# beehive-lab/GPULlama3.java

Measured on AMD Instinct MI355X. Metric: tg128 tok/s (llama-bench), Llama-3-8B Q8_0, higher is better.
Workload: dtype i8; 1 GPU; Llama-3-8B-random Q8_0 random-weight GGUF-layout model, tg128 at depth 0 (one step = 128 decode tokens, logits D2H inside the timed region); parallelism=single GPU, ranks=1, ctx=648

## Files before the change

### gpullama3.java_amd/csrc/gl3_api.hip

```cpp
#include <chrono>
#include <cstdio>
#include <cstdlib>
#include <cstring>
#include <vector>

#include "gl3_ctx.h"
#include "gl3_batch_plan.h"
#include "gl3_decode_kernels.h"
#include "gl3_rowlane_kernels.h"
#include "gl3_veclane_kernels.h"
#include "gl3_moe_kernels.h"
#include "gl3_kv_copy.h"

using namespace gl3;

static std::string g_create_err;

static double now_ms() {
    return std::chrono::duration<double, std::milli>(std::chrono::steady_clock::now().time_since_epoch()).count();
}


static size_t matvec_smem(int pro, int epi, const Q8Mat& w) {
    const int nm = epi == EPI_SWIGLU ? 2 : 1;
    return (size_t)w.ng * 4 * 32 + (size_t)w.ng * 4 * 4 + (pro == PRO_RMS ? (size_t)(w.k + 32) * 4 : 0) + (size_t)2 * nm * w.ng * 64 * 4 + 128;
}

#include <hip/hip_ext.h>
template <typename K>
static void launch_mv(gl3_ctx* ctx, K kernel, int wgs, int threads, size_t smem, const MatvecArgs& a) {
    if (ctx->prof_ev0) hipExtLaunchKernelGGL(kernel, dim3(wgs), dim3(threads), (uint32_t)smem, ctx->stream, ctx->prof_ev0, ctx->prof_ev1, 0, a);
    else hipLaunchKernelGGL(kernel, dim3(wgs), dim3(threads), smem, ctx->stream, a);
}

template <int PRO, int EPI>
static void launch_matvec_t(gl3_ctx* ctx, const MatvecArgs& a, int wgs, size_t smem, bool nt) {
    if (a.tp) { launch_mv(ctx, matvec_q8t_kernel<PRO, EPI, true, 4, false, true>, wgs, mv_threads(4), smem, a); return; }
    if (nt) launch_mv(ctx, matvec_q8t_kernel<PRO, EPI, true>, wgs, mv_threads(4), smem, a);
    else launch_mv(ctx, matvec_q8t_kernel<PRO, EPI, false>, wgs, mv_threads(4), smem, a);
}

template <int PRO, int EPI>
static hipError_t allow_big_lds() {
    hipError_t e = hipFuncSetAttribute((const void*)matvec_q8t_kernel<PRO, EPI, true>, hipFuncAttributeMaxDynamicSharedMemorySize, 160 * 1024 - 256);
    if (e != hipSuccess) return e;
    e = hipFuncSetAttribute((const void*)matvec_q8t_kernel<PRO, EPI, true, 4, false, true>, hipFuncAttributeMaxDynamicSharedMemorySize, 160 * 1024 - 256);
    if (e != hipSuccess) return e;
    return hipFuncSetAttribute((const void*)matvec_q8t_kernel<PRO, EPI, false>, hipFuncAttributeMaxDynamicSharedMemorySize, 160 * 1024 - 256);
}

static void launch_matvec(gl3_ctx* ctx, int pro, int epi, const Q8Mat& w, const Q8Mat* w2, const float* x,
                          const float* norm_w, float* out, const float* resid_in, float out_scale = 1.0f, const TpRec* tp = nullptr) {
    if (w.fmt != GL3_TYPE_Q8_0) {
        hipStream_t s = ctx->stream;
        static const bool vl_rms = env_flag("GL3_VL_RMS", true);
        static const bool ksplit_on = env_flag("GL3_VLQ", true);
        const bool ksplit_type = ksplit_on && w.vl && (w.fmt == GL3_FMT_Q8V || w.fmt == GL3_TYPE_Q4_0);
        const long vl_waves = (long)((w.rows + 7) / 8) * (epi == EPI_SWIGLU ? 2 : 1);
        const bool fuse_rms = pro == PRO_RMS && w.vl && vl_rms && vl_rms_fusable(w.k) && epi != EPI_RESID && !(ksplit_type && vl_waves <= 512);
        if (pro == PRO_RMS && !fuse_rms) {
            const size_t sm = (size_t)(w.k + 32) * 4 + ss_scratch_bytes(w.k) + 64;
            hipLaunchKernelGGL(rmsnorm_f32_kernel, dim3(1), dim3(256), sm, s, x, w.k, norm_w, ctx->d.rms_eps, ctx->xn);
            x = ctx->xn;
        }
        if (w.vl) {
            VlArgs v{};
            v.w = w.w; v.w2 = w2 ? w2->w : nullptr; v.rows = w.rows; v.k = w.k; v.x = x; v.out = out; v.resid_in = resid_in; v.out_scale = out_scale;
            v.tp = tp;
            const dim3 vg(((w.rows + 7) / 8 + VL_WAVES - 1) / VL_WAVES), vb(64 * VL_WAVES);
            const size_t vs = vl_smem_bytes(w.k);
            if (fuse_rms) {
                v.norm_w = norm_w; v.eps = ctx->d.rms_eps;
                const dim3 rg(((w.rows + 7) / 8 + VL_RMS_WAVES - 1) / VL_RMS_WAVES), rb(64 * VL_RMS_WAVES);
                const size_t rs = vl_rms_smem_bytes(w.k);
#define GL3_VLR(WT_) \
                do { \
                    if (epi == EPI_STORE) hipLaunchKernelGGL((matvec_vl_kernel<WT_, EPI_STORE, true, VL_RMS_WAVES>), rg, rb, rs, s, v); \
                    else hipLaunchKernelGGL((matvec_vl_kernel<WT_, EPI_SWIGLU, true, VL_RMS_WAVES>), rg, rb, rs, s, v); \
                } while (0)
                if (w.fmt == GL3_TYPE_F16 && (ctx->d.flags & GL3_FLAG_VECTOR_512)) {
                    if (epi == EPI_STORE) hipLaunchKernelGGL((matvec_vl_kernel<WT_F16, EPI_STORE, true, VL_RMS_WAVES, 512>), rg, rb, rs, s, v);
                    else hipLaunchKernelGGL((matvec_vl_kernel<WT_F16, EPI_SWIGLU, true, VL_RMS_WAVES, 512>), rg, rb, rs, s, v);
                }
                else if (w.fmt == GL3_TYPE_F16) GL3_VLR(WT_F16); else if (w.fmt == GL3_FMT_Q8V) GL3_VLR(WT_Q8_0); else GL3_VLR(WT_Q4_0);
#undef GL3_VLR
                return;
            }
#define GL3_VL(WT_) \
            do { \
                if (epi == EPI_STORE) hipLaunchKernelGGL((matvec_vl_kernel<WT_, EPI_STORE>), vg, vb, vs, s, v); \
                else if (epi == EPI_RESID) hipLaunchKernelGGL((matvec_vl_kernel<WT_, EPI_RESID>), vg, vb, vs, s, v); \
                else hipLaunchKernelGGL((matvec_vl_kernel<WT_, EPI_SWIGLU>), vg, vb, vs, s, v); \
            } while (0)
            static const bool ksplit = env_flag("GL3_VLQ", true);
#define GL3_VLQ_E(WT_, MAXW_) \
            do { \
                const size_t qs = vq_smem_bytes<WT_, MAXW_>(w.k, epi == EPI_SWIGLU ? 2 : 1, nw); \
                if (epi == EPI_STORE) hipLaunchKernelGGL((matvec_vlq_kernel<WT_, EPI_STORE, MAXW_>), qg, qb, qs, s, v); \
                else if (epi == EPI_RESID) hipLaunchKernelGGL((matvec_vlq_kernel<WT_, EPI_RESID, MAXW_>), qg, qb, qs, s, v); \
                else hipLaunchKernelGGL((matvec_vlq_kernel<WT_, EPI_SWIGLU, MAXW_>), qg, qb, qs, s, v); \
            } while (0)
#define GL3_VLQ(WT_) \
            do { \
                const int ngroups = (w.rows + 7) / 8, nw = vq_waves<WT_>(w.k, epi == EPI_SWIGLU ? 2 : 1, ngroups); \
                const dim3 qg(ngroups), qb(64 * nw); \
                if (nw == 16) GL3_VLQ_E(WT_, 16); else GL3_VLQ_E(WT_, 8); \
            } while (0)
            if (w.fmt == GL3_TYPE_F16 && (ctx->d.flags & GL3_FLAG_VECTOR_512)) {
                if (epi == EPI_STORE) hipLaunchKernelGGL((matvec_vl_kernel<WT_F16, EPI_STORE, false, VL_WAVES, 512>), vg, vb, vs, s, v);
                else if (epi == EPI_RESID) hipLaunchKernelGGL((matvec_vl_kernel<WT_F16, EPI_RESID, false, VL_WAVES, 512>), vg, vb, vs, s, v);
                else hipLaunchKernelGGL((matvec_vl_kernel<WT_F16, EPI_SWIGLU, false, VL_WAVES, 512>), vg, vb, vs, s, v);
            }
            else if (w.fmt == GL3_TYPE_F16) GL3_VL(WT_F16);
            else if (w.fmt == GL3_FMT_Q8V) { if (ksplit) GL3_VLQ(WT_Q8_0); else GL3_VL(WT_Q8_0); }
            else { if (ksplit) GL3_VLQ(WT_Q4_0); else GL3_VL(WT_Q4_0); }
#undef GL3_VLQ
#undef GL3_VLQ_E
#undef GL3_VL
            return;
        }
        RlArgs a{};
        a.w = w.w; a.w2 = w2 ? w2->w : nullptr; a.rows = w.rows; a.k = w.k; a.x = x; a.out = out; a.resid_in = resid_in; a.out_scale = out_scale;
        const dim3 grid((w.rows + 63) / 64);
        const size_t sm = rl_smem_bytes(w.k, epi);
#define GL3_RL(WT_) \
        do { \
            if (epi == EPI_STORE) hipLaunchKernelGGL((matvec_rl_kernel<WT_, EPI_STORE>), grid, dim3(RL_THREADS), sm, s, a); \
            else if (epi == EPI_RESID) hipLaunchKernelGGL((matvec_rl_kernel<WT_, EPI_RESID>), grid, dim3(RL_THREADS), sm, s, a); \
            else hipLaunchKernelGGL((matvec_rl_kernel<WT_, EPI_SWIGLU>), grid, dim3(RL_THREADS), sm, s, a); \
        } while (0)
        if (w.fmt == GL3_TYPE_F16) GL3_RL(WT_F16); else GL3_RL(WT_Q4_0);
#undef GL3_RL
        return;
    }
    static const bool nt = env_flag("GL3_NT", true);
    static const int max_wgs = getenv("GL3_WGS") ? atoi(getenv("GL3_WGS")) : 512;
    MatvecArgs a{};
    a.w = w.w; a.w2 = w2 ? w2->w : nullptr; a.rows = w.rows; a.k = w.k; a.ng = w.ng; a.nstrips = w.nstrips;
    a.x = x; a.norm_w = norm_w; a.eps = ctx->d.rms_eps; a.out = out; a.resid_in = resid_in; a.out_scale = out_scale;
    a.tp = tp;
    const int wgs = w.nstrips < max_wgs ? w.nstrips : max_wgs;
    const size_t smem = matvec_smem(pro, epi, w);
    if (pro == PRO_RMS && epi == EPI_STORE) launch_matvec_t<PRO_RMS, EPI_STORE>(ctx, a, wgs, smem, nt);
    else if (pro == PRO_QUANT && epi == EPI_RESID) {
        static const int wide_max = getenv("GL3_WIDE_STRIPS") ? atoi(getenv("GL3_WIDE_STRIPS")) : 256;
        if (w.nstrips <= wide_max && nt && tp)
            launch_mv(ctx, matvec_q8t_kernel<PRO_QUANT, EPI_RESID, true, 8, false, true>, wgs, mv_threads(8), smem, a);
        else if (w.nstrips <= wide_max && nt)
            launch_mv(ctx, matvec_q8t_kernel<PRO_QUANT, EPI_RESID, true, 8>, wgs, mv_threads(8), smem, a);
        else launch_matvec_t<PRO_QUANT, EPI_RESID>(ctx, a, wgs, smem, nt);
    }
    else launch_matvec_t<PRO_RMS, EPI_SWIGLU>(ctx, a, wgs, smem, nt);
}

static void launch_matvec_sel(gl3_ctx* ctx, int layer, int which, const Q8Mat& stack, const Q8Mat* stack2, int rows, const float* x,
                              const float* norm_w, float* out, int shared_rows) {
    const gl3_model_desc& d = ctx->d;
    static const int max_wgs = getenv("GL3_WGS") ? atoi(getenv("GL3_WGS")) : 512;
    Q8Mat sub = stack;
    sub.rows = rows; sub.nstrips = rows / 16;
    MatvecArgs a{};
    a.w = stack.w; a.w2 = stack2 ? stack2->w : nullptr; a.rows = rows; a.k = stack.k; a.ng = stack.ng; a.nstrips = sub.nstrips;
    a.x = x; a.norm_w = norm_w; a.eps = d.rms_eps; a.out = out; a.resid_in = nullptr; a.out_scale = 1.0f;
    a.moe = reinterpret_cast<const MoeSlots*>(ctx->moe_slots) + (size_t)layer * 3 + which;
    const int slots = d.n_experts_used + (which == 0 ? (shared_rows + rows - 1) / rows : 0);
    const int wgs = sub.nstrips < max_wgs ? sub.nstrips : max_wgs;
    const dim3 grid(wgs, slots);
    if (which != 2) hipLaunchKernelGGL((matvec_q8t_kernel<PRO_RMS, EPI_SWIGLU, true, 4, true>), grid, dim3(mv_threads(4)), matvec_smem(PRO_RMS, EPI_SWIGLU, sub), ctx->stream, a);
    else hipLaunchKernelGGL((matvec_q8t_kernel<PRO_QUANT, EPI_RESID, true, 4, true>), grid, dim3(mv_threads(4)), matvec_smem(PRO_QUANT, EPI_RESID, sub), ctx->stream, a);
}

static int32_t moe_build_slots(gl3_ctx* ctx) {
    const gl3_model_desc& d = ctx->d;
    std::vector<MoeSlots> h((size_t)d.n_layers * 3);
    for (int l = 0; l < d.n_layers; ++l) {
        const gl3_layer& L = ctx->layers[l];
        MoeSlots gu{};
        gu.sel = ctx->moe_sel; gu.sel_stride = (size_t)(d.moe_hidden / 16) * L.gate_exps.ng * TILE_BYTES;
        gu.x_slot_stride = 0; gu.out_slot_stride = d.moe_hidden; gu.n_sel = d.n_experts_used;
        gu.sh_rows = L.w1.rows; gu.sh_w = L.w1.w; gu.sh_w2 = L.w3.w; gu.sh_out = ctx->hb;
        h[(size_t)l * 3 + 0] = gu;
        gu.sh_rows = 0; gu.sh_w = gu.sh_w2 = nullptr; gu.sh_out = nullptr;
        h[(size_t)l * 3 + 1] = gu;
        MoeSlots dn{};
        dn.sel = ctx->moe_sel; dn.sel_stride = (size_t)(d.dim / 16) * L.down_exps.ng * TILE_BYTES;
        dn.x_slot_stride = d.moe_hidden; dn.out_slot_stride = d.dim; dn.n_sel = d.n_experts_used;
        h[(size_t)l * 3 + 2] = dn;
    }
    GL3_HIP(hipMalloc(&ctx->moe_slots, h.size() * sizeof(MoeSlots)));
    GL3_HIP(hipMemcpy(ctx->moe_slots, h.data(), h.size() * sizeof(MoeSlots), hipMemcpyHostToDevice));
    return GL3_OK;
}

struct Prof {
    gl3_ctx* ctx; gl3_kernel_times* kt; size_t n = 0; std::vector<int> klass;
    bool ext = false;
    void begin(int k, uint64_t bytes, bool single_kernel = false) {
        if (!kt) return;
        if (ctx->ev.size() < 2 * (n + 1)) {
            ctx->ev.resize(2 * (n + 1));
            hipEventCreate(&ctx->ev[2 * n]); hipEventCreate(&ctx->ev[2 * n + 1]);
        }
        ext = single_kernel;
        if (ext) { ctx->prof_ev0 = ctx->ev[2 * n]; ctx->prof_ev1 = ctx->ev[2 * n + 1]; }
        else hipEventRecord(ctx->ev[2 * n], ctx->stream);
        klass.push_back(k); kt->launches[k]++; kt->bytes[k] += bytes;
    }
    void end() {
        if (!kt) return;
        if (ext) ctx->prof_ev0 = ctx->prof_ev1 = nullptr;
        else hipEventRecord(ctx->ev[2 * n + 1], ctx->stream);
        ++n;
    }
    void collect() {
        if (!kt) return;
        hipStreamSynchronize(ctx->stream);
        for (size_t i = 0; i < n; ++i) {
            float ms = 0; hipEventElapsedTime(&ms, ctx->ev[2 * i], ctx->ev[2 * i + 1]);
            kt->ms[klass[i]] += ms;
        }
    }
};

static uint64_t mv_bytes(const Q8Mat& w) { return w.algo_bytes() + (uint64_t)w.k * 4 + (uint64_t)w.rows * 4; }

static void enqueue_moe_ffn(gl3_ctx* ctx, int l, Prof& pr) {
    gl3_layer& L = ctx->layers[l];
    const gl3_model_desc& d = ctx->d;
    hipStream_t s = ctx->stream;
    const int E = d.n_experts, topk = d.n_experts_used, mh = d.moe_hidden;
// ... 354 lines not shown
    ctx->q_dim = d.n_heads * d.head_size; ctx->kv_dim = d.n_kv_heads * d.head_size;
    ctx->heads_l = d.n_heads / tp; ctx->kv_heads_l = d.n_kv_heads / tp;
    ctx->q_dim_l = ctx->heads_l * d.head_size; ctx->kv_dim_l = ctx->kv_heads_l * d.head_size;
    ctx->hidden_l = d.hidden / tp; ctx->vocab_l = d.vocab / tp; ctx->dim_l = d.dim / tp;
    ctx->n_tsplit = (d.ctx + ATT_TT - 1) / ATT_TT;
    ctx->wo_replicated = tp > 1 && !env_flag("GL3_TP_SPLIT_WO", false) && (d.max_batch <= 1 || d.dim % (32 * tp) == 0);
    ctx->wo_rows = ctx->wo_replicated ? d.dim : ctx->dim_l;
    ctx->use_rccl = tp > 1 || (d.flags & GL3_FLAG_FORCE_RCCL);

#define TRY(x) do { int32_t r_ = (x); if (r_ != GL3_OK) return bail(r_, ""); } while (0)
#define TRYHIP(x) do { hipError_t e_ = (x); if (e_ != hipSuccess) return bail(e_ == hipErrorOutOfMemory ? GL3_E_OOM : GL3_E_HIP, std::string(#x) + ": " + hipGetErrorString(e_)); } while (0)
    TRYHIP(hipSetDevice(d.device));
    TRYHIP(hipStreamCreateWithFlags(&ctx->stream, hipStreamNonBlocking));
    TRY(alloc_mat(ctx, ctx->emb, d.vocab, d.dim));
    ctx->layers.resize(d.n_layers);
    for (auto& L : ctx->layers) {
        TRY(alloc_mat(ctx, L.wqkv, ctx->q_dim_l + 2 * ctx->kv_dim_l, d.dim));
        TRY(alloc_mat(ctx, L.wo, ctx->wo_rows, ctx->q_dim));
        TRY(alloc_mat(ctx, L.w1, ctx->hidden_l, d.dim));
        TRY(alloc_mat(ctx, L.w3, ctx->hidden_l, d.dim));
        TRY(alloc_mat(ctx, L.w2, ctx->dim_l, d.hidden));
        TRY(dmalloc(ctx, &L.attn_norm, d.dim));
        TRY(dmalloc(ctx, &L.ffn_norm, d.dim));
        if (d.arch == GL3_ARCH_QWEN3) { TRY(dmalloc(ctx, &L.qnorm, d.head_size)); TRY(dmalloc(ctx, &L.knorm, d.head_size)); }
        if (d.arch == GL3_ARCH_QWEN2 || moe) { TRY(dmalloc(ctx, &L.bq, ctx->q_dim_l)); TRY(dmalloc(ctx, &L.bk, ctx->kv_dim_l)); TRY(dmalloc(ctx, &L.bv, ctx->kv_dim_l)); }
        if (moe) {
            TRY(alloc_mat(ctx, L.gate_exps, d.n_experts * d.moe_hidden, d.dim));
            TRY(alloc_mat(ctx, L.up_exps, d.n_experts * d.moe_hidden, d.dim));
            TRY(alloc_mat(ctx, L.down_exps, d.n_experts * d.dim, d.moe_hidden));
            TRY(dmalloc(ctx, &L.gate_inp, (size_t)d.n_experts * d.dim));
            TRY(dmalloc(ctx, &L.gate_inp_shexp, d.dim));
        }
    }
    if (moe) {
        TRY(dmalloc(ctx, &ctx->moe_logits, d.n_experts));
        TRY(dmalloc(ctx, &ctx->moe_w, d.n_experts_used + 1));
        TRY(dmalloc(ctx, &ctx->moe_sel, d.n_experts_used + 1));
        TRY(dmalloc(ctx, &ctx->moe_hb, (size_t)d.n_experts_used * d.moe_hidden));
        TRY(dmalloc(ctx, &ctx->moe_y, (size_t)(d.n_experts_used + 1) * d.dim));
        TRYHIP(hipMemset(ctx->moe_sel, 0, sizeof(int) * (d.n_experts_used + 1)));
        TRYHIP(hipFuncSetAttribute((const void*)matvec_q8t_kernel<PRO_RMS, EPI_SWIGLU, true, 4, true>, hipFuncAttributeMaxDynamicSharedMemorySize, 160 * 1024 - 256));
        TRYHIP(hipFuncSetAttribute((const void*)matvec_q8t_kernel<PRO_QUANT, EPI_RESID, true, 4, true>, hipFuncAttributeMaxDynamicSharedMemorySize, 160 * 1024 - 256));
        TRYHIP(hipFuncSetAttribute((const void*)moe_router_kernel, hipFuncAttributeMaxDynamicSharedMemorySize, 160 * 1024 - 256));
    }
    TRY(dmalloc(ctx, &ctx->out_norm, d.dim));
    ctx->kv_seq_stride = (size_t)d.n_layers * d.ctx * ctx->kv_dim_l;
    const size_t kvn = ctx->kv_seq_stride * ctx->n_seqs;
    TRY(dmalloc(ctx, &ctx->kcache, kvn));
    TRY(dmalloc(ctx, &ctx->vcache, kvn + (size_t)PVT * ctx->kv_dim_l));
    TRYHIP(hipMemset(ctx->kcache, 0, kvn * 4));
    TRYHIP(hipMemset(ctx->vcache, 0, (kvn + (size_t)PVT * ctx->kv_dim_l) * 4));
    if (ctx->n_seqs > 1) TRY(dmalloc(ctx, &ctx->kv_copy_dst, ctx->n_seqs));
    TRY(dmalloc(ctx, &ctx->xn, d.dim));
    TRY(dmalloc(ctx, &ctx->qkv, ctx->q_dim_l + 2 * ctx->kv_dim_l));
    if (ctx->use_rccl) {
        if (tp > GL3_MAX_TP) return bail(GL3_E_UNSUPPORTED, "tp_size above 16");
        TRY(gl3_tp_arena_alloc(ctx));
        ctx->x = (float*)(ctx->arena.base + ctx->arena.off[GB_X]); ctx->xb = (float*)(ctx->arena.base + ctx->arena.off[GB_XB]);
        ctx->hb = (float*)(ctx->arena.base + ctx->arena.off[GB_HB]); ctx->logits = (float*)(ctx->arena.base + ctx->arena.off[GB_LOGITS]);
    } else {
        TRY(dmalloc(ctx, &ctx->x, d.dim));
        TRY(dmalloc(ctx, &ctx->xb, ctx->q_dim));
        TRY(dmalloc(ctx, &ctx->hb, d.hidden));
        TRY(dmalloc(ctx, &ctx->logits, d.vocab));
    }
    TRY(dmalloc(ctx, &ctx->att, (size_t)ctx->heads_l * ((d.ctx + 3) & ~3)));
    TRY(dmalloc(ctx, &ctx->att_t, attn_att_t_floats(ctx->kv_heads_l, d.n_heads / d.n_kv_heads, (d.ctx + 3) & ~3)));
    TRYHIP(hipMemset(ctx->att_t, 0, attn_att_t_floats(ctx->kv_heads_l, d.n_heads / d.n_kv_heads, (d.ctx + 3) & ~3) * 4));
    TRY(dmalloc(ctx, &ctx->att_tmax, (size_t)ctx->heads_l * ctx->n_tsplit));
    TRY(dmalloc(ctx, &ctx->att_sums, (size_t)ctx->heads_l));
    if (moe) TRY(moe_build_slots(ctx));
    TRYHIP((allow_big_lds<PRO_RMS, EPI_STORE>()));
    TRYHIP((allow_big_lds<PRO_QUANT, EPI_RESID>()));
    TRYHIP((allow_big_lds<PRO_RMS, EPI_SWIGLU>()));
    {
        ctx->fused_attn_ok = d.head_size % 4 == 0 && attn_head_smem(d.head_size) <= 150 * 1024 && !env_flag("GL3_NO_FUSED_ATTN", false);
        if (ctx->fused_attn_ok) {
            hipError_t ae = hipSuccess;
            attn_head_dispatch(d.head_size, [&](auto kern) { ae = hipFuncSetAttribute((const void*)kern, hipFuncAttributeMaxDynamicSharedMemorySize, 160 * 1024 - 256); });
            TRYHIP(ae);
        }
    }
    TRYHIP(hipFuncSetAttribute((const void*)matvec_q8t_kernel<PRO_QUANT, EPI_RESID, true, 8>, hipFuncAttributeMaxDynamicSharedMemorySize, 160 * 1024 - 256));
#define GL3_RL_LDS(...) TRYHIP(hipFuncSetAttribute((const void*)matvec_rl_kernel<__VA_ARGS__>, hipFuncAttributeMaxDynamicSharedMemorySize, 160 * 1024 - 256))
    GL3_RL_LDS(WT_F16, EPI_STORE); GL3_RL_LDS(WT_F16, EPI_RESID); GL3_RL_LDS(WT_F16, EPI_SWIGLU);
    GL3_RL_LDS(WT_Q4_0, EPI_STORE); GL3_RL_LDS(WT_Q4_0, EPI_RESID); GL3_RL_LDS(WT_Q4_0, EPI_SWIGLU);
#undef GL3_RL_LDS
    TRYHIP(hipFuncSetAttribute((const void*)rmsnorm_f32_kernel, hipFuncAttributeMaxDynamicSharedMemorySize, 160 * 1024 - 256));
    TRYHIP(hipFuncSetAttribute((const void*)attn_scores_kernel, hipFuncAttributeMaxDynamicSharedMemorySize, 128 * 1024));
    TRYHIP(hipFuncSetAttribute((const void*)attn_scores_loop_kernel<128>, hipFuncAttributeMaxDynamicSharedMemorySize, 128 * 1024));
    TRYHIP(hipFuncSetAttribute((const void*)attn_scores_loop_kernel<64>, hipFuncAttributeMaxDynamicSharedMemorySize, 128 * 1024));
    TRYHIP(hipFuncSetAttribute((const void*)attn_softmax_pv_kernel, hipFuncAttributeMaxDynamicSharedMemorySize, 150 * 1024));
    TRYHIP(hipFuncSetAttribute((const void*)attn_sum_kernel, hipFuncAttributeMaxDynamicSharedMemorySize, (int)attn_sum_smem()));
    TRYHIP(hipFuncSetAttribute((const void*)attn_pv_kernel, hipFuncAttributeMaxDynamicSharedMemorySize, (int)attn_pv_smem()));
    {
        const char* wv = getenv("GL3_ATTN_WINDOW");
        int wmax = wv && *wv ? atoi(wv) : 16384;
        if (wmax < PV_ROWS || wmax % PV_ROWS != 0 || wmax > 16384) return bail(GL3_E_ARG, "GL3_ATTN_WINDOW must be a multiple of 1024 between 1024 and 16384");
        ctx->attn_win = d.ctx <= wmax ? ((d.ctx + 3) & ~3) : wmax;
        const char* mv = getenv("GL3_ATTN_MID");
        ctx->attn_mid = mv && *mv ? atoi(mv) : 768;
    }
    TRY(dmalloc(ctx, &ctx->dyn, GL3_DYN_INTS));
    ctx->dyn_cur = ctx->dyn;
    TRY(dmalloc(ctx, &ctx->argmax, 2 + 2 * AMX_WGS));
    TRYHIP(hipMemset(ctx->argmax, 0, (2 + 2 * AMX_WGS) * sizeof(int)));
    if (d.flags & GL3_FLAG_LAYER_TAPS) TRY(dmalloc(ctx, &ctx->taps, (size_t)d.n_layers * d.dim));
    TRYHIP(hipHostMalloc((void**)&ctx->h_dyn, GL3_DYN_INTS * sizeof(int)));
    TRYHIP(hipHostMalloc((void**)&ctx->h_logits, (size_t)d.vocab * 4));
    TRYHIP(hipHostMalloc((void**)&ctx->h_argmax, sizeof(int)));
    {
        const bool int8_path = d.weight_type == GL3_TYPE_Q8_0 && !(d.flags & GL3_FLAG_F32_ACTIVATION);
        const bool vl_path = !int8_path && !(d.flags & GL3_FLAG_SCALAR_DOT);
        if (d.max_batch > 1 && (int8_path || vl_path)) TRY(gl3_prefill_alloc(ctx));
    }
    if (getenv("GL3_DEBUG_ALLOC")) {
        fprintf(stderr, "[gl3 alloc] ctx %p emb %p (+%zu) kcache %p vcache %p (%zu floats) x %p qkv %p xb %p hb %p logits %p att %p xn %p\n", (void*)ctx, (void*)ctx->emb.w,
                ctx->emb.bytes(), (void*)ctx->kcache, (void*)ctx->vcache, kvn, (void*)ctx->x, (void*)ctx->qkv, (void*)ctx->xb, (void*)ctx->hb, (void*)ctx->logits, (void*)ctx->att, (void*)ctx->xn);
        for (size_t l = 0; l < ctx->layers.size(); ++l) {
            const gl3_layer& L = ctx->layers[l];
            fprintf(stderr, "[gl3 alloc]   layer %zu wqkv %p (+%zu) wo %p (+%zu) w1 %p (+%zu) w3 %p w2 %p (+%zu)\n", l, (void*)L.wqkv.w, L.wqkv.bytes(), (void*)L.wo.w, L.wo.bytes(),
                    (void*)L.w1.w, L.w1.bytes(), (void*)L.w3.w, (void*)L.w2.w, L.w2.bytes());
        }
    }
    TRYHIP(hipDeviceSynchronize());
#undef TRY
#undef TRYHIP
    ctx->plan_ms = now_ms() - t0;
    *out = ctx;
    return GL3_OK;
}

void gl3_destroy(gl3_ctx* ctx) {
    if (!ctx) return;
    hipSetDevice(ctx->d.device);
    if (ctx->stream) hipStreamSynchronize(ctx->stream);
    if (ctx->graph_exec) hipGraphExecDestroy(ctx->graph_exec);
    if (ctx->graph_exec_s) hipGraphExecDestroy(ctx->graph_exec_s);
    if (ctx->graph_exec_m) hipGraphExecDestroy(ctx->graph_exec_m);
    if (ctx->graph_m) hipGraphDestroy(ctx->graph_m);
    if (ctx->graph_s) hipGraphDestroy(ctx->graph_s);
    if (ctx->graph) hipGraphDestroy(ctx->graph);
    if (ctx->comm) ncclCommDestroy(ctx->comm);
    gl3_prefill_free(ctx);
    gl3_sample_free(ctx);
    gl3_score_free(ctx);
    for (auto e : ctx->ev) hipEventDestroy(e);
    auto f = [](void* p) { if (p) hipFree(p); };
    f(ctx->emb.w);
    if (ctx->wcls_owned) f(ctx->wcls.w);
    for (auto& L : ctx->layers) {
        f(L.wqkv.w); f(L.wo.w); f(L.w1.w); f(L.w3.w); f(L.w2.w);
        f(L.attn_norm); f(L.ffn_norm); f(L.qnorm); f(L.knorm); f(L.bq); f(L.bk); f(L.bv);
        f(L.gate_exps.w); f(L.up_exps.w); f(L.down_exps.w); f(L.gate_inp); f(L.gate_inp_shexp);
    }
    f(ctx->moe_logits); f(ctx->moe_w); f(ctx->moe_sel); f(ctx->moe_hb); f(ctx->moe_y); f(ctx->moe_slots); f(ctx->tp_recs);
    f(ctx->out_norm); f(ctx->rope_cr); f(ctx->rope_ci); f(ctx->kcache); f(ctx->vcache); f(ctx->kv_copy_dst); f(ctx->xn); f(ctx->qkv);
    if (!ctx->arena.base) { f(ctx->x); f(ctx->xb); f(ctx->hb); f(ctx->logits); }
    gl3_tp_arena_free(ctx);
    f(ctx->att); f(ctx->att_t); f(ctx->att_tmax); f(ctx->att_sums); f(ctx->dyn); f(ctx->dyn_seq); f(ctx->argmax); f(ctx->taps); f(ctx->staging);
    for (auto& pr : ctx->pinned) hipHostUnregister(pr.first);
    ctx->pinned.clear();
    if (ctx->h_dyn) hipHostFree(ctx->h_dyn);
    if (ctx->h_logits) hipHostFree(ctx->h_logits);
    if (ctx->h_argmax) hipHostFree(ctx->h_argmax);
    if (ctx->stream) hipStreamDestroy(ctx->stream);
// ... 821 lines not shown
```

### gpullama3.java_amd/csrc/gl3_decode_kernels.h

```cpp
#pragma once
#include <hip/hip_runtime.h>
#include <stdint.h>

#include "gl3_seqsum.h"

namespace gl3 {

constexpr int TILE_BYTES = 2176;
constexpr int MV_AUX = 4;
__host__ __device__ constexpr int mv_threads(int npw) { return 64 * (npw + MV_AUX); }

enum { PRO_RMS = 0, PRO_QUANT = 1 };
enum { EPI_STORE = 0, EPI_RESID = 1, EPI_SWIGLU = 2 };

typedef float v4f __attribute__((ext_vector_type(4)));

#ifdef GL3_MV_TIMING
__device__ long long gl3_mv_stamp[32];
#define ATT_STAMP(i) do { if (blockIdx.x == 0 && threadIdx.x == 0) gl3_mv_stamp[i] = wall_clock64(); } while (0)
#define MV_STAMP(i, cond) do { if (blockIdx.x == 0 && (cond)) gl3_mv_stamp[i] = clock64(); } while (0)
#define PV_T(...) __VA_ARGS__
#else
#define PV_T(...)
#define MV_STAMP(i, cond)
#define ATT_STAMP(i)
#endif

constexpr int TPF_MAX_PEERS = 15;
struct TpWait {
    const uint32_t* flags;
    const uint32_t* step;
    uint32_t* err;
    int mul, add, tp, me;
    unsigned spin_limit;
};
struct TpPush {
    uint32_t* ticket;
    const uint32_t* step;
    int mul, add, npeers;
    long delta[TPF_MAX_PEERS];
    uint32_t* flag[TPF_MAX_PEERS];
};
struct TpRec { TpWait w; TpPush p; };

__device__ __forceinline__ void tp_wait(const TpWait& w) {
    const uint32_t need = (__hip_atomic_load(w.step, __ATOMIC_RELAXED, __HIP_MEMORY_SCOPE_AGENT) - 1u) * (uint32_t)w.mul + (uint32_t)w.add;
    const int lane = threadIdx.x & 63;
    const bool mine = lane < w.tp && lane != w.me;
    unsigned spins = 0;
    for (;;) {
        const bool ok = !mine || (int32_t)(__hip_atomic_load(w.flags + (mine ? lane : 0), __ATOMIC_RELAXED, __HIP_MEMORY_SCOPE_SYSTEM) - need) >= 0;
        if (__builtin_amdgcn_ballot_w64(!ok) == 0) break;
        __builtin_amdgcn_s_sleep(8);
        if (++spins > w.spin_limit) { if (lane == 0) __hip_atomic_store(w.err, 1u, __ATOMIC_RELAXED, __HIP_MEMORY_SCOPE_SYSTEM); break; }
    }
    __builtin_amdgcn_fence(__ATOMIC_ACQUIRE, "");
}
__device__ __forceinline__ void tp_push_store(const TpPush& p, float* own, float v) {
    for (int j = 0; j < p.npeers; ++j)
        *reinterpret_cast<float*>(reinterpret_cast<uint8_t*>(own) + p.delta[j]) = v;
}
__device__ __forceinline__ void tp_publish(const TpPush& p, unsigned total) {
    asm volatile("s_waitcnt vmcnt(0)" ::: "memory");
    if ((threadIdx.x & 63) != 0) return;
    const unsigned ticket = __hip_atomic_fetch_add(p.ticket, 1u, __ATOMIC_RELAXED, __HIP_MEMORY_SCOPE_AGENT);
    if (ticket != total - 1) return;
    __hip_atomic_store(p.ticket, 0u, __ATOMIC_RELAXED, __HIP_MEMORY_SCOPE_AGENT);
    const uint32_t k = (__hip_atomic_load(p.step, __ATOMIC_RELAXED, __HIP_MEMORY_SCOPE_AGENT) - 1u) * (uint32_t)p.mul + (uint32_t)p.add;
    __threadfence_system();
    for (int j = 0; j < p.npeers; ++j) __hip_atomic_store(p.flag[j], k, __ATOMIC_RELEASE, __HIP_MEMORY_SCOPE_SYSTEM);
}

static __global__ __launch_bounds__(64) void tp_wait_kernel(const TpRec* r) { tp_wait(r->w); }

struct MatvecArgs {
    const uint8_t* w;
    const uint8_t* w2;
    int rows;
    int k;
    int ng;
    int nstrips;
    const float* x;
    const float* norm_w;
    float eps;
    float* out;
    const float* resid_in;
    float out_scale;
    const struct MoeSlots* moe;
    const TpRec* tp;
};

struct MoeSlots {
    const int* sel;
    size_t sel_stride;
    int x_slot_stride, out_slot_stride;
    int n_sel, sh_rows;
    const uint8_t* sh_w;
    const uint8_t* sh_w2;
    float* sh_out;
};

__device__ __forceinline__ void lds_barrier() { asm volatile("s_waitcnt lgkmcnt(0)\n\ts_barrier" ::: "memory"); }

struct LdsBarrier { __device__ __forceinline__ void operator()() const { lds_barrier(); } };

__device__ __forceinline__ float h2f(uint16_t h) { return (float)__builtin_bit_cast(_Float16, h); }

// ... 33 lines not shown
    asm("v_mul_f32 %0, %1, %2" : "=v"(r) : "v"(a), "v"(b));
    return r;
}

__device__ __forceinline__ float seq_sum_lds_ring(const float* v, int n, float start = 0.f) {
    float s = start;
    const int G = n >> 4;
    int i = 0;
    if (G >= 3) {
        float4 a0, a1, a2, a3, b0, b1, b2, b3, c0, c1, c2, c3;
#define SSR_LD(G_, V0_, V1_, V2_, V3_) do { const float* q_ = v + 16 * min((G_), G - 1); V0_ = *reinterpret_cast<const float4*>(q_); \
        V1_ = *reinterpret_cast<const float4*>(q_ + 4); V2_ = *reinterpret_cast<const float4*>(q_ + 8); V3_ = *reinterpret_cast<const float4*>(q_ + 12); } while (0)
#define SSR_ADD(V0_, V1_, V2_, V3_) do { s = seq_add4<false>(s, V0_); s = seq_add4<false>(s, V1_); s = seq_add4<false>(s, V2_); s = seq_add4<false>(s, V3_); } while (0)
        SSR_LD(0, a0, a1, a2, a3); SSR_LD(1, b0, b1, b2, b3); SSR_LD(2, c0, c1, c2, c3);
        int g = 0;
        for (; g + 3 <= G; g += 3) {
            SSR_ADD(a0, a1, a2, a3); SSR_LD(g + 3, a0, a1, a2, a3); __builtin_amdgcn_sched_barrier(0);
            SSR_ADD(b0, b1, b2, b3); SSR_LD(g + 4, b0, b1, b2, b3); __builtin_amdgcn_sched_barrier(0);
            SSR_ADD(c0, c1, c2, c3); SSR_LD(g + 5, c0, c1, c2, c3); __builtin_amdgcn_sched_barrier(0);
        }
        if (g < G) { SSR_ADD(a0, a1, a2, a3); ++g; }
        if (g < G) { SSR_ADD(b0, b1, b2, b3); ++g; }
#undef SSR_ADD
#undef SSR_LD
        i = 16 * G;
    }
    for (; i + 4 <= n; i += 4) s = seq_add4<false>(s, *reinterpret_cast<const float4*>(v + i));
    for (; i < n; ++i) s = s + v[i];
    return s;
}

__device__ __forceinline__ uint32_t quantize_quad_pack(float4 v, float& qs_out) {
    float amax = fmaxf(fmaxf(fabsf(v.x), fabsf(v.y)), fmaxf(fabsf(v.z), fabsf(v.w)));
    amax = fmaxf(amax, __builtin_bit_cast(float, __builtin_amdgcn_update_dpp(0, __builtin_bit_cast(int, amax), 0xB1, 0xf, 0xf, false)));
    amax = fmaxf(amax, __builtin_bit_cast(float, __builtin_amdgcn_update_dpp(0, __builtin_bit_cast(int, amax), 0x4E, 0xf, 0xf, false)));
    amax = fmaxf(amax, __builtin_bit_cast(float, __builtin_amdgcn_update_dpp(0, __builtin_bit_cast(int, amax), 0x141, 0xf, 0xf, false)));
    const float qs = amax / 127.0f;
    const float ainv = qs != 0.f ? 1.0f / qs : 0.f;
    const float s0 = v.x * ainv, s1 = v.y * ainv, s2 = v.z * ainv, s3 = v.w * ainv;
    const int q0 = (int)(s0 + copysignf(0.5f, s0)), q1 = (int)(s1 + copysignf(0.5f, s1));
    const int q2 = (int)(s2 + copysignf(0.5f, s2)), q3 = (int)(s3 + copysignf(0.5f, s3));
    qs_out = (float)(_Float16)qs;
    return (uint32_t)(q0 & 0xFF) | ((uint32_t)(q1 & 0xFF) << 8) | ((uint32_t)(q2 & 0xFF) << 16) | ((uint32_t)(q3 & 0xFF) << 24);
}

__device__ __forceinline__ void quantize_quad(float4 v, int qd, uint8_t* xq, float* xs) {
    float qs;
    const uint32_t packed = quantize_quad_pack(v, qs);
    *reinterpret_cast<uint32_t*>(xq + 4 * qd) = packed;
    if ((qd & 7) == 0) xs[qd >> 3] = qs;
}

__device__ __forceinline__ size_t bdq_offset(int qd, int tok, int tslots) {
    const int blk = qd >> 3, qi = qd & 7, c = qi >> 1;
    const int g = ((c & 1) << 1) | (c >> 1);
    return ((size_t)(blk >> 1) * tslots + tok) * 64 + 16 * g + 8 * (blk & 1) + 4 * (qi & 1);
}
__device__ __forceinline__ size_t bds_offset(int blk, int tok, int tslots) { return ((size_t)(blk >> 2) * tslots + tok) * 4 + (blk & 3); }

__device__ __forceinline__ int dot32(const int4& a0, const int4& a1, const int4& b0, const int4& b1) {
    int s = 0;
    s = __builtin_amdgcn_sdot4(a0.x, b0.x, s, false); s = __builtin_amdgcn_sdot4(a0.y, b0.y, s, false);
    s = __builtin_amdgcn_sdot4(a0.z, b0.z, s, false); s = __builtin_amdgcn_sdot4(a0.w, b0.w, s, false);
    s = __builtin_amdgcn_sdot4(a1.x, b1.x, s, false); s = __builtin_amdgcn_sdot4(a1.y, b1.y, s, false);
    s = __builtin_amdgcn_sdot4(a1.z, b1.z, s, false); s = __builtin_amdgcn_sdot4(a1.w, b1.w, s, false);
    return s;
}

template <bool NT>
__device__ __forceinline__ int4 ld16(const uint8_t* p) {
    typedef int v4i __attribute__((ext_vector_type(4)));
    v4i v;
    if (NT) v = __builtin_nontemporal_load(reinterpret_cast<const v4i*>(p));
    else v = *reinterpret_cast<const v4i*>(p);
    int4 r; r.x = v.x; r.y = v.y; r.z = v.z; r.w = v.w;
    return r;
}
template <bool NT>
__device__ __forceinline__ uint16_t ld2(const uint8_t* p) {
    if (NT) return __builtin_nontemporal_load(reinterpret_cast<const uint16_t*>(p));
    return *reinterpret_cast<const uint16_t*>(p);
}

template <int PRO, int EPI, bool NT, int NPW = 4, bool SEL = false, bool TPF = false>
__global__ __launch_bounds__(mv_threads(NPW), NPW == 4 ? 4 : 2) void matvec_q8t_kernel(const MatvecArgs a_in) {
    MatvecArgs a = a_in;
    if (SEL) {
        const int slot = blockIdx.y;
        const MoeSlots m = *a.moe;
        if (slot < m.n_sel) {
            const size_t woff = (size_t)m.sel[slot] * m.sel_stride;
            a.w += woff;
            if (a.w2) a.w2 += woff;
            a.x += (size_t)slot * m.x_slot_stride;
            a.out += (size_t)slot * m.out_slot_stride;
        } else {
            const int c = slot - m.n_sel;
            const size_t woff = (size_t)c * m.sel_stride;
            a.w = m.sh_w + woff;
            a.w2 = m.sh_w2 ? m.sh_w2 + woff : nullptr;
            a.out = m.sh_out + (size_t)c * a.rows;
            const int left = m.sh_rows - c * a.rows;
            if (left < a.rows) { a.rows = left; a.nstrips = (left + 15) / 16; }
        }
    }
    constexpr int MV_PRODUCERS = NPW;
    extern __shared__ __attribute__((aligned(16))) uint8_t smem[];
    constexpr int NM = (EPI == EPI_SWIGLU) ? 2 : 1;
    constexpr int CH = (NM == 1) ? 8 : 4;
    const int t = threadIdx.x, lane = t & 63, wave = t >> 6;
    const int nb4 = a.ng * 4;
    uint8_t* xq = smem;
    float* xs = reinterpret_cast<float*>(smem + (size_t)nb4 * 32);
    float* xf = xs + nb4;
    float* pbuf = xf + (PRO == PRO_RMS ? a.k + 32 : 0);
    float* red = pbuf + (size_t)2 * NM * a.ng * 64;
    int* sync_w = reinterpret_cast<int*>(red + 4);
    const size_t strip_bytes = (size_t)a.ng * TILE_BYTES;
    MV_STAMP(0, t == 0);
    if (t < 2) sync_w[t] = 0;

    if (wave < MV_PRODUCERS) {
        const int nt = (a.ng - wave + MV_PRODUCERS - 1) / MV_PRODUCERS;
        uint16_t sc[NM][CH];
        int4 lo[NM][CH], hi[NM][CH];
        auto issue = [&](int strip, int i0) {
#pragma unroll
            for (int u = 0; u < CH; ++u) {
                if (i0 + u < nt) {
                    const int g = wave + (i0 + u) * MV_PRODUCERS;
#pragma unroll
                    for (int m = 0; m < NM; ++m) {
                        const uint8_t* p = (m == 0 ? a.w : a.w2) + (size_t)strip * strip_bytes + (size_t)g * TILE_BYTES;
                        sc[m][u] = ld2<NT>(p + 2 * lane);
                        lo[m][u] = ld16<NT>(p + 128 + 16 * lane);
                        hi[m][u] = ld16<NT>(p + 1152 + 16 * lane);
                    }
                }
            }
        };
        auto compute = [&](int i0, float* pb) {
#pragma unroll
            for (int u = 0; u < CH; ++u) {
                if (i0 + u < nt) {
                    const int g = wave + (i0 + u) * MV_PRODUCERS;
                    const int xb = 4 * g + (lane >> 4);
                    const int4 xlo = *reinterpret_cast<const int4*>(xq + 32 * xb);
                    const int4 xhi = *reinterpret_cast<const int4*>(xq + 32 * xb + 16);
                    const float xsc = xs[xb];
#pragma unroll
                    for (int m = 0; m < NM; ++m) {
                        const int isum = dot32(lo[m][u], hi[m][u], xlo, xhi);
                        pb[(size_t)m * a.ng * 64 + g * 64 + lane] = (float)isum * (h2f(sc[m][u]) * xsc);
                    }
                }
            }
        };
        int strip = blockIdx.x;
        __syncthreads();
        if (strip < a.nstrips) issue(strip, 0);
        while (__hip_atomic_load(&sync_w[1], __ATOMIC_RELAXED, __HIP_MEMORY_SCOPE_WORKGROUP) == 0) __builtin_amdgcn_s_sleep(2);
        __builtin_amdgcn_fence(__ATOMIC_ACQUIRE, "workgroup");
        MV_STAMP(3, t == 0);
        int it = 0;
        for (; strip < a.nstrips; strip += gridDim.x, ++it) {
            float* pb = pbuf + (size_t)(it & 1) * NM * a.ng * 64;
            for (int i0 = 0; i0 < nt; i0 += CH) {
                if (it != 0 || i0 != 0) issue(strip, i0);
                compute(i0, pb);
            }
            MV_STAMP(4 + 2 * it, t == 0 && it < 4);
            __syncthreads();
            MV_STAMP(5 + 2 * it, t == 0 && it < 4);
        }
        return;
    }

    __builtin_amdgcn_s_setprio(3);
    const int ta = t - 64 * MV_PRODUCERS;
    const int nquads = a.k >> 2;
    float scale = 1.0f;
    constexpr int NXV = (PRO == PRO_RMS) ? 5 : 14;
    float4 nwv[5], xv[NXV];
    if (!TPF) {
#pragma unroll
        for (int i = 0; i < NXV; ++i) xv[i] = *reinterpret_cast<const float4*>(a.x + 4 * min(ta + 256 * i, nquads - 1));
    }
    if (PRO == PRO_RMS) {
#pragma unroll
        for (int i = 0; i < 5; ++i) nwv[i] = *reinterpret_cast<const float4*>(a.norm_w + 4 * min(ta + 256 * i, nquads - 1));
    }
    __syncthreads();
    if (TPF) {
        if (a.tp->w.flags) tp_wait(a.tp->w);
#pragma unroll
        for (int i = 0; i < NXV; ++i) xv[i] = *reinterpret_cast<const float4*>(a.x + 4 * min(ta + 256 * i, nquads - 1));
    }
    SubBarrier aux_sync{&sync_w[0], MV_AUX, 0};
    if (PRO == PRO_RMS) {
        if (nquads <= NXV * 256) {
#pragma unroll
            for (int i = 0; i < NXV; ++i) { const int qd = ta + 256 * i; if (qd < nquads) *reinterpret_cast<float4*>(xf + 4 * qd) = xv[i]; }
        } else {
            for (int qd = ta; qd < nquads; qd += 256)
                *reinterpret_cast<float4*>(xf + 4 * qd) = *reinterpret_cast<const float4*>(a.x + 4 * qd);
        }
        if (ta < 32) xf[a.k + ta] = 0.f;
        aux_sync();
        MV_STAMP(1, ta == 0);
        float ss;
        if ((size_t)2 * NM * a.ng * 64 * 4 >= ss_scratch_bytes(a.k) && a.k >= 1024 && a.k <= 5120) {
            ss = exact_sumsq_lds(xf, a.k, reinterpret_cast<uint8_t*>(pbuf), ta, aux_sync);
        } else {
            if (wave == MV_PRODUCERS) {
                const float s1 = seq_sum_lds<true>(xf, a.k);
                if (lane == 0) red[0] = s1;
            }
            aux_sync();
            ss = red[0];
        }
        MV_STAMP(2, ta == 0);
        ss /= (float)a.k;
        ss += a.eps;
        scale = (float)(1.0 / sqrt((double)ss));
    }
    for (int b = (a.k >> 5) + ta; b < nb4; b += 256) {
        xs[b] = 0.f;
        const int4 z = {0, 0, 0, 0};
        *reinterpret_cast<int4*>(xq + 32 * b) = z;
        *reinterpret_cast<int4*>(xq + 32 * b + 16) = z;
    }
    if (nquads <= NXV * 256) {
#pragma unroll
        for (int i = 0; i < NXV; ++i) {
            const int qd = ta + 256 * i;
            if (qd < nquads) {
                float4 v = xv[i];
                if (PRO == PRO_RMS) {
                    const float4 w = nwv[i];
                    v.x = w.x * (scale * v.x); v.y = w.y * (scale * v.y); v.z = w.z * (scale * v.z); v.w = w.w * (scale * v.w);
                }
                quantize_quad(v, qd, xq, xs);
            }
        }
    } else {
        for (int qd = ta; qd < nquads; qd += 256) {
            float4 v = *reinterpret_cast<const float4*>(a.x + 4 * qd);
            if (PRO == PRO_RMS) {
                const float4 w = *reinterpret_cast<const float4*>(a.norm_w + 4 * qd);
                v.x = w.x * (scale * v.x); v.y = w.y * (scale * v.y); v.z = w.z * (scale * v.z); v.w = w.w * (scale * v.w);
            }
            quantize_quad(v, qd, xq, xs);
        }
    }
    aux_sync();
    if (ta == 0) __hip_atomic_store(&sync_w[1], 1, __ATOMIC_RELEASE, __HIP_MEMORY_SCOPE_WORKGROUP);
    if (wave != MV_PRODUCERS) return;

    int it = 0;
    for (int strip = blockIdx.x; strip < a.nstrips; strip += gridDim.x, ++it) {
        __syncthreads();
        MV_STAMP(16 + 2 * it, lane == 0 && it < 4);
        const float* pb = pbuf + (size_t)(it & 1) * NM * a.ng * 64;
        v4f acc[NM];
#pragma unroll
        for (int m = 0; m < NM; ++m) acc[m] = (v4f){0.f, 0.f, 0.f, 0.f};
        int g = 0;
        for (; g + 8 <= a.ng; g += 8) {
            float av[NM][8];
#pragma unroll
            for (int m = 0; m < NM; ++m)
#pragma unroll
                for (int u = 0; u < 8; ++u) av[m][u] = pb[(size_t)m * a.ng * 64 + (g + u) * 64 + lane];
#pragma unroll
            for (int u = 0; u < 8; ++u)
#pragma unroll
                for (int m = 0; m < NM; ++m) acc[m] = __builtin_amdgcn_mfma_f32_16x16x4f32(av[m][u], 1.0f, acc[m], 0, 0, 0);
        }
        for (; g < a.ng; ++g)
#pragma unroll
            for (int m = 0; m < NM; ++m)
                acc[m] = __builtin_amdgcn_mfma_f32_16x16x4f32(pb[(size_t)m * a.ng * 64 + g * 64 + lane], 1.0f, acc[m], 0, 0, 0);
        MV_STAMP(17 + 2 * it, lane == 0 && it < 4);
        if ((lane & 15) < 4) {
            const int r = lane & 3;
            const int row = strip * 16 + 4 * (lane >> 4) + r;
            if (row < a.rows) {
                const float v0 = r == 0 ? acc[0][0] : r == 1 ? acc[0][1] : r == 2 ? acc[0][2] : acc[0][3];
                float res;
                if (EPI == EPI_STORE) res = v0 * a.out_scale;
                if (EPI == EPI_RESID) res = a.resid_in ? a.resid_in[row] + v0 * a.out_scale : v0 * a.out_scale;
                if (EPI == EPI_SWIGLU) {
                    const float v1 = r == 0 ? acc[NM - 1][0] : r == 1 ? acc[NM - 1][1] : r == 2 ? acc[NM - 1][2] : acc[NM - 1][3];
                    const float gte = v0 / (float)(1.0 + exp(-(double)v0));
                    res = gte * v1;
                }
                a.out[row] = res;
                if (TPF) tp_push_store(a.tp->p, a.out + row, res);
            }
        }
    }
    if (TPF && a.tp->p.npeers) tp_publish(a.tp->p, gridDim.x);
}

static __global__ __launch_bounds__(256) void embed_q8t_kernel(const uint8_t* __restrict__ emb, int ng, int dim,
                                                         const int* __restrict__ dyn, float* __restrict__ x, float emb_scale,
                                                         const TpRec* tp = nullptr, uint32_t* step = nullptr) {
    if (step) {
        const uint32_t s = *step;
        __syncthreads();
        if (threadIdx.x == 0) *step = s + 1;
        if (tp) {
            TpWait w = tp->w;
            const uint32_t need = s * (uint32_t)w.mul;
            const int lane = threadIdx.x & 63;
            const bool mine = lane < w.tp && lane != w.me;
            unsigned spins = 0;
            for (;;) {
                const bool ok = !mine || (int32_t)(__hip_atomic_load(w.flags + (mine ? lane : 0), __ATOMIC_RELAXED, __HIP_MEMORY_SCOPE_SYSTEM) - need) >= 0;
                if (__builtin_amdgcn_ballot_w64(!ok) == 0) break;
                __builtin_amdgcn_s_sleep(8);
                if (++spins > w.spin_limit) { if (lane == 0) __hip_atomic_store(w.err, 1u, __ATOMIC_RELAXED, __HIP_MEMORY_SCOPE_SYSTEM); break; }
            }
        }
    }
    const int token = dyn[0];
    const uint8_t* strip = emb + (size_t)(token >> 4) * ng * TILE_BYTES;
    const int i16 = token & 15;
    for (int i = threadIdx.x; i < dim; i += 256) {
        const int b = i >> 5, j = i & 31;
        const uint8_t* p = strip + (size_t)(b >> 2) * TILE_BYTES;
        const int l = i16 + 16 * (b & 3);
        const float d = h2f(*reinterpret_cast<const uint16_t*>(p + 2 * l));
        const int8_t q = (int8_t)p[(j < 16 ? 128 : 1152) + 16 * l + (j & 15)];
        x[i] = ((float)q * d) * emb_scale;
    }
}

struct AttnArgs {
    const float* qkv;
    float* kcache;
    float* vcache;
    const float* rope_cr;
    const float* rope_ci;
    const float* qnorm;
    const float* knorm;
    const float* bq;
    const float* bk;
    const float* bv;
    const int* dyn;
    float* att;
    float* xb;
    int n_heads, n_kv_heads, hs, q_dim, kv_dim, ctx;
    float eps;
    int arch;
    const int* seqv;
    const int* posv;
    size_t seq_stride;
    int qkv_stride, xb_stride;
    float att_mul;
    int win;
    int att_stride;
    float* att_t;
    float* tmax;
    float* sums;
    int group;
    uint8_t* xq_out; float* xs_out; int xq_slots;
    const TpRec* tp;
};

__device__ __forceinline__ void rope_head(float* v, int hs, const float* cr, const float* ci, int arch, int t0, int nthreads) {
    const int half = hs >> 1;
    for (int i = t0; i < half; i += nthreads) {
        const float fcr = cr[i], fci = ci[i];
        const int i0 = arch == 0 ? 2 * i : i, i1 = arch == 0 ? 2 * i + 1 : i + half;
        const float v0 = v[i0], v1 = v[i1];
        v[i0] = v0 * fcr - v1 * fci;
        v[i1] = v0 * fci + v1 * fcr;
    }
}

__device__ __forceinline__ void head_rmsnorm_wave(float* v, const float* __restrict__ w, int hs, float eps, int lane) {
    float ss = seq_sum_lds<true>(v, hs);
// ... 823 lines not shown
```

Baseline: 470.3 tok/s.

## Stream matvec partial sums to consumer wave in segments via LDS barriers

Adds a SEGS variant of the Q8 matvec kernel in which producer waves signal the consumer (MFMA reduction) wave after each chunk batch with lds_barrier, instead of one full __syncthreads per strip. The consumer reduces partials segment by segment, overlapping the reduction with producers' remaining loads. The host selects this variant when the group count exceeds one segment. It also adds per-workgroup timing stamps that compile only under profiling. The risks are more barriers per strip and barrier-count mismatches between producer and consumer waves.

Result: faster. 478.0 tok/s, median of 6 (+1.6%).

```diff
diff --git a/gpullama3.java_amd/csrc/gl3_api.hip b/gpullama3.java_amd/csrc/gl3_api.hip
--- a/gpullama3.java_amd/csrc/gl3_api.hip
+++ b/gpullama3.java_amd/csrc/gl3_api.hip
@@ -35,8 +35,14 @@
 
 template <int PRO, int EPI>
 static void launch_matvec_t(gl3_ctx* ctx, const MatvecArgs& a, int wgs, size_t smem, bool nt) {
-    if (a.tp) { launch_mv(ctx, matvec_q8t_kernel<PRO, EPI, true, 4, false, true>, wgs, mv_threads(4), smem, a); return; }
-    if (nt) launch_mv(ctx, matvec_q8t_kernel<PRO, EPI, true>, wgs, mv_threads(4), smem, a);
+    const bool segs = a.ng > mv_seg_groups(4, EPI);
+    if (a.tp) {
+        if (segs) launch_mv(ctx, matvec_q8t_kernel<PRO, EPI, true, 4, false, true, true>, wgs, mv_threads(4), smem, a);
+        else launch_mv(ctx, matvec_q8t_kernel<PRO, EPI, true, 4, false, true>, wgs, mv_threads(4), smem, a);
+        return;
+    }
+    if (nt && segs) launch_mv(ctx, matvec_q8t_kernel<PRO, EPI, true, 4, false, false, true>, wgs, mv_threads(4), smem, a);
+    else if (nt) launch_mv(ctx, matvec_q8t_kernel<PRO, EPI, true>, wgs, mv_threads(4), smem, a);
     else launch_mv(ctx, matvec_q8t_kernel<PRO, EPI, false>, wgs, mv_threads(4), smem, a);
 }
 
@@ -45,6 +51,10 @@
     hipError_t e = hipFuncSetAttribute((const void*)matvec_q8t_kernel<PRO, EPI, true>, hipFuncAttributeMaxDynamicSharedMemorySize, 160 * 1024 - 256);
     if (e != hipSuccess) return e;
     e = hipFuncSetAttribute((const void*)matvec_q8t_kernel<PRO, EPI, true, 4, false, true>, hipFuncAttributeMaxDynamicSharedMemorySize, 160 * 1024 - 256);
+    if (e != hipSuccess) return e;
+    e = hipFuncSetAttribute((const void*)matvec_q8t_kernel<PRO, EPI, true, 4, false, false, true>, hipFuncAttributeMaxDynamicSharedMemorySize, 160 * 1024 - 256);
+    if (e != hipSuccess) return e;
+    e = hipFuncSetAttribute((const void*)matvec_q8t_kernel<PRO, EPI, true, 4, false, true, true>, hipFuncAttributeMaxDynamicSharedMemorySize, 160 * 1024 - 256);
     if (e != hipSuccess) return e;
     return hipFuncSetAttribute((const void*)matvec_q8t_kernel<PRO, EPI, false>, hipFuncAttributeMaxDynamicSharedMemorySize, 160 * 1024 - 256);
 }
@@ -144,8 +154,13 @@
     if (pro == PRO_RMS && epi == EPI_STORE) launch_matvec_t<PRO_RMS, EPI_STORE>(ctx, a, wgs, smem, nt);
     else if (pro == PRO_QUANT && epi == EPI_RESID) {
         static const int wide_max = getenv("GL3_WIDE_STRIPS") ? atoi(getenv("GL3_WIDE_STRIPS")) : 256;
-        if (w.nstrips <= wide_max && nt && tp)
+        const bool segs = w.ng > mv_seg_groups(8, EPI_RESID);
+        if (w.nstrips <= wide_max && nt && tp && segs)
+            launch_mv(ctx, matvec_q8t_kernel<PRO_QUANT, EPI_RESID, true, 8, false, true, true>, wgs, mv_threads(8), smem, a);
+        else if (w.nstrips <= wide_max && nt && tp)
             launch_mv(ctx, matvec_q8t_kernel<PRO_QUANT, EPI_RESID, true, 8, false, true>, wgs, mv_threads(8), smem, a);
+        else if (w.nstrips <= wide_max && nt && segs)
+            launch_mv(ctx, matvec_q8t_kernel<PRO_QUANT, EPI_RESID, true, 8, false, false, true>, wgs, mv_threads(8), smem, a);
         else if (w.nstrips <= wide_max && nt)
             launch_mv(ctx, matvec_q8t_kernel<PRO_QUANT, EPI_RESID, true, 8>, wgs, mv_threads(8), smem, a);
         else launch_matvec_t<PRO_QUANT, EPI_RESID>(ctx, a, wgs, smem, nt);
@@ -666,6 +681,8 @@
         }
     }
     TRYHIP(hipFuncSetAttribute((const void*)matvec_q8t_kernel<PRO_QUANT, EPI_RESID, true, 8>, hipFuncAttributeMaxDynamicSharedMemorySize, 160 * 1024 - 256));
+    TRYHIP(hipFuncSetAttribute((const void*)matvec_q8t_kernel<PRO_QUANT, EPI_RESID, true, 8, false, false, true>, hipFuncAttributeMaxDynamicSharedMemorySize, 160 * 1024 - 256));
+    TRYHIP(hipFuncSetAttribute((const void*)matvec_q8t_kernel<PRO_QUANT, EPI_RESID, true, 8, false, true, true>, hipFuncAttributeMaxDynamicSharedMemorySize, 160 * 1024 - 256));
 #define GL3_RL_LDS(...) TRYHIP(hipFuncSetAttribute((const void*)matvec_rl_kernel<__VA_ARGS__>, hipFuncAttributeMaxDynamicSharedMemorySize, 160 * 1024 - 256))
     GL3_RL_LDS(WT_F16, EPI_STORE); GL3_RL_LDS(WT_F16, EPI_RESID); GL3_RL_LDS(WT_F16, EPI_SWIGLU);
     GL3_RL_LDS(WT_Q4_0, EPI_STORE); GL3_RL_LDS(WT_Q4_0, EPI_RESID); GL3_RL_LDS(WT_Q4_0, EPI_SWIGLU);
diff --git a/gpullama3.java_amd/csrc/gl3_decode_kernels.h b/gpullama3.java_amd/csrc/gl3_decode_kernels.h
--- a/gpullama3.java_amd/csrc/gl3_decode_kernels.h
+++ b/gpullama3.java_amd/csrc/gl3_decode_kernels.h
@@ -12,6 +12,8 @@
 
 enum { PRO_RMS = 0, PRO_QUANT = 1 };
 enum { EPI_STORE = 0, EPI_RESID = 1, EPI_SWIGLU = 2 };
+__host__ __device__ constexpr int mv_ch(int epi) { return epi == EPI_SWIGLU ? 4 : 8; }
+__host__ __device__ constexpr int mv_seg_groups(int npw, int epi) { return npw * mv_ch(epi); }
 
 typedef float v4f __attribute__((ext_vector_type(4)));
 
@@ -20,9 +22,15 @@
 #define ATT_STAMP(i) do { if (blockIdx.x == 0 && threadIdx.x == 0) gl3_mv_stamp[i] = wall_clock64(); } while (0)
 #define MV_STAMP(i, cond) do { if (blockIdx.x == 0 && (cond)) gl3_mv_stamp[i] = clock64(); } while (0)
 #define PV_T(...) __VA_ARGS__
+constexpr int MV_WG_STAMPS = 1024;
+__device__ unsigned long long gl3_mv_wg_stamp[MV_WG_STAMPS][8];
+#define MV_WG_TIME(v) v = (unsigned long long)wall_clock64()
+#define MV_WG_PUT(s, v, cond) do { if (blockIdx.x < MV_WG_STAMPS && blockIdx.y == 0 && (cond)) atomicMax(&gl3_mv_wg_stamp[blockIdx.x][s], v); } while (0)
 #else
 #define PV_T(...)
 #define MV_STAMP(i, cond)
+#define MV_WG_TIME(v)
+#define MV_WG_PUT(s, v, cond)
 #define ATT_STAMP(i)
 #endif
 
@@ -222,7 +230,7 @@
     return *reinterpret_cast<const uint16_t*>(p);
 }
 
-template <int PRO, int EPI, bool NT, int NPW = 4, bool SEL = false, bool TPF = false>
+template <int PRO, int EPI, bool NT, int NPW = 4, bool SEL = false, bool TPF = false, bool SEGS = false>
 __global__ __launch_bounds__(mv_threads(NPW), NPW == 4 ? 4 : 2) void matvec_q8t_kernel(const MatvecArgs a_in) {
     MatvecArgs a = a_in;
     if (SEL) {
@@ -247,9 +255,11 @@
     constexpr int MV_PRODUCERS = NPW;
     extern __shared__ __attribute__((aligned(16))) uint8_t smem[];
     constexpr int NM = (EPI == EPI_SWIGLU) ? 2 : 1;
-    constexpr int CH = (NM == 1) ? 8 : 4;
+    constexpr int CH = mv_ch(EPI);
     const int t = threadIdx.x, lane = t & 63, wave = t >> 6;
     const int nb4 = a.ng * 4;
+    constexpr int SEG = mv_seg_groups(NPW, EPI);
+    const int nbatch = SEGS ? ((a.ng + NPW - 1) / NPW + CH - 1) / CH : 1;
     uint8_t* xq = smem;
     float* xs = reinterpret_cast<float*>(smem + (size_t)nb4 * 32);
     float* xf = xs + nb4;
@@ -258,6 +268,8 @@
     int* sync_w = reinterpret_cast<int*>(red + 4);
     const size_t strip_bytes = (size_t)a.ng * TILE_BYTES;
     MV_STAMP(0, t == 0);
+    PV_T(unsigned long long wg_t0 = 0, wg_t1 = 0, wg_t2 = 0;)
+    MV_WG_TIME(wg_t0);
     if (t < 2) sync_w[t] = 0;
 
     if (wave < MV_PRODUCERS) {
@@ -308,11 +320,22 @@
             for (int i0 = 0; i0 < nt; i0 += CH) {
                 if (it != 0 || i0 != 0) issue(strip, i0);
                 compute(i0, pb);
-            }
-            MV_STAMP(4 + 2 * it, t == 0 && it < 4);
-            __syncthreads();
+                if (SEGS) {
+                    MV_STAMP(4 + 2 * it, t == 0 && it < 4 && i0 + CH >= nt);
+                    MV_WG_TIME(wg_t1);
+                    lds_barrier();
+                }
+            }
+            if (SEGS) {
+                for (int b = (nt + CH - 1) / CH; b < nbatch; ++b) lds_barrier();
+            } else {
+                MV_STAMP(4 + 2 * it, t == 0 && it < 4);
+                MV_WG_TIME(wg_t1);
+                __syncthreads();
+            }
             MV_STAMP(5 + 2 * it, t == 0 && it < 4);
         }
+        MV_WG_PUT(0, wg_t0, t == 0); MV_WG_PUT(1, wg_t1, lane == 0);
         return;
     }
 
@@ -399,29 +422,34 @@
 
     int it = 0;
     for (int strip = blockIdx.x; strip < a.nstrips; strip += gridDim.x, ++it) {
-        __syncthreads();
-        MV_STAMP(16 + 2 * it, lane == 0 && it < 4);
         const float* pb = pbuf + (size_t)(it & 1) * NM * a.ng * 64;
         v4f acc[NM];
 #pragma unroll
         for (int m = 0; m < NM; ++m) acc[m] = (v4f){0.f, 0.f, 0.f, 0.f};
-        int g = 0;
-        for (; g + 8 <= a.ng; g += 8) {
-            float av[NM][8];
-#pragma unroll
-            for (int m = 0; m < NM; ++m)
-#pragma unroll
-                for (int u = 0; u < 8; ++u) av[m][u] = pb[(size_t)m * a.ng * 64 + (g + u) * 64 + lane];
-#pragma unroll
-            for (int u = 0; u < 8; ++u)
-#pragma unroll
-                for (int m = 0; m < NM; ++m) acc[m] = __builtin_amdgcn_mfma_f32_16x16x4f32(av[m][u], 1.0f, acc[m], 0, 0, 0);
-        }
-        for (; g < a.ng; ++g)
-#pragma unroll
-            for (int m = 0; m < NM; ++m)
-                acc[m] = __builtin_amdgcn_mfma_f32_16x16x4f32(pb[(size_t)m * a.ng * 64 + g * 64 + lane], 1.0f, acc[m], 0, 0, 0);
+        for (int b = 0; b < nbatch; ++b) {
+            if (SEGS) lds_barrier(); else __syncthreads();
+            MV_STAMP(16 + 2 * it, lane == 0 && it < 4 && b == nbatch - 1);
+            MV_WG_TIME(wg_t1);
+            int g = b * SEG;
+            const int ge = SEGS ? min(g + SEG, a.ng) : a.ng;
+            for (; g + 8 <= ge; g += 8) {
+                float av[NM][8];
+#pragma unroll
+                for (int m = 0; m < NM; ++m)
+#pragma unroll
+                    for (int u = 0; u < 8; ++u) av[m][u] = pb[(size_t)m * a.ng * 64 + (g + u) * 64 + lane];
+#pragma unroll
+                for (int u = 0; u < 8; ++u)
+#pragma unroll
+                    for (int m = 0; m < NM; ++m) acc[m] = __builtin_amdgcn_mfma_f32_16x16x4f32(av[m][u], 1.0f, acc[m], 0, 0, 0);
+            }
+            for (; g < ge; ++g)
+#pragma unroll
+                for (int m = 0; m < NM; ++m)
+                    acc[m] = __builtin_amdgcn_mfma_f32_16x16x4f32(pb[(size_t)m * a.ng * 64 + g * 64 + lane], 1.0f, acc[m], 0, 0, 0);
+        }
         MV_STAMP(17 + 2 * it, lane == 0 && it < 4);
+        MV_WG_TIME(wg_t2);
         if ((lane & 15) < 4) {
             const int r = lane & 3;
             const int row = strip * 16 + 4 * (lane >> 4) + r;
@@ -439,6 +467,9 @@
                 if (TPF) tp_push_store(a.tp->p, a.out + row, res);
             }
         }
+        PV_T(asm volatile("s_waitcnt vmcnt(0)" ::: "memory");)
+        MV_WG_TIME(wg_t0);
+        MV_WG_PUT(2, wg_t1, lane == 0); MV_WG_PUT(3, wg_t2, lane == 0); MV_WG_PUT(4, wg_t0, lane == 0);
     }
     if (TPF && a.tp->p.npeers) tp_publish(a.tp->p, gridDim.x);
 }
```
